# ygahounzo/h-NUMO

Measured on AMD Instinct MI355X. Metric: DG element-updates/sec (all layers, per RK stage), higher is better.
Workload: dtype f64; 1 GPU; dg25L3: double-gyre-3 25x25 elements per GPU, N=4, 3 layers, N_btp=20, kstages=5; elements=625, elements_per_gpu=625, nlayers=3, nop=4, parallelism=single, summation=reference

## Files before the change

### h-numo_amd/csrc/engine.hip

```cpp
#include <hip/hip_runtime.h>
#include <hip/hip_ext.h>

#include <rccl/rccl.h>

#include <algorithm>
#include <cmath>
#include <condition_variable>
#include <cstdio>
#include <cstring>
#include <mutex>
#include <string>
#include <thread>
#include <type_traits>
#include <vector>

#include "../../include/hnumo_engine.h"
#include "engine_internal.h"
#include "setup_plan.h"
#include "sample_plan.h"
#include "float_plan.h"
#include "kernels_bcl.hip"
#include "kernels_btp.hip"
#include "kernels_lapq.hip"
#include "kernels_diag.hip"
// ... 46 lines not shown
  DevMesh m{};
  hnumo_params p{};
  int nelem, npoin, npq, nface, ngl, nq, L, P, Q, K;
  size_t FQ, FN;
  std::vector<void *> allocs;
  double *basis, *qstat, *nstat, *fstat, *fnstat, *alpha, *tau_wind;
  int *iconn;
  std::vector<double> ssprk_a, ssprk_beta;
  double *q, *qb, *qp, *q2, *qp2, *qbp, *qf, *qf2, *qfa, *dpp2;
  double *qbuf[4], *gtrace[2];
  double *qcoef, *ncoef, *fcoef, *fncoef, *dpp_graduv, *dpprime_visc, *gdpp_face;
  double *ecoef, *efcoef;
  double *qstatE, *nstatE, *efstat;
  std::vector<int> fslotA;
  double *qacc, *facc, *nacc, *gfacc, *tau_wind_ave;
  double *slmf, *slmf_face, *dpp, *fmass, *fcons, *momL, *lapf, *rhs;
  int *neg_flag, *h_neg;
  hipGraph_t graph = nullptr;
  hipGraphExec_t graph_exec = nullptr;
  bool resident = false, uploaded = false, alloc_failed = false;
  hipEvent_t ev0 = nullptr, ev1 = nullptr;
  hipEvent_t evk0 = nullptr, evk1 = nullptr;
  bool capturing = false, kernel_events = false, no_graph = false;
  int graph_env = -1;
  int summation = HNUMO_SUM_REFERENCE;
  unsigned long long *stage_prof = nullptr;
  int stage_dbg = 0;
  int stage_nb = 0;
  bool bcl_big = false;
  bool acc_zero = false;
  bool persistent_ok[2] = {false, false};
  bool regacc[2] = {false, false};
  TraceGranule *gtr[2] = {nullptr, nullptr};
  unsigned long long *epoch = nullptr;
  unsigned *sub_done = nullptr;
  unsigned *sub_arrive = nullptr;
  unsigned *steps_done = nullptr, *h_steps = nullptr;
  int occ_blocks[2] = {0, 0}, occ_ncu = 0, probe_ok[2] = {-1, -1};
  int persist_pad = 0;
  int persist_guard = 3;
  int persist_aborts = 0;
  bool persist_suspended = false;
  int persist_wait = 0, persist_backoff = 1, persist_reprobes = 0, persist_recovered = 0;
  unsigned long long *dbg_abort_epoch = nullptr;
  StageArgs *d_stages[2] = {nullptr, nullptr};
  bool face_halo = false;
  int NS = 0;
  using FNbr = SetupPlan::FNbr;
  std::vector<FNbr> fnb;
  int *d_sface = nullptr;
  double *bx_sbuf = nullptr, *bx_rbuf = nullptr;
  size_t bx_per_max = 0;
  int *d_elB = nullptr, *d_elI = nullptr;
  int nB = 0, nI = 0;
  double *cdef = nullptr;
  bool emu_frozen = false;
  int xseq = 0;
  struct Frozen {
    const void *key;
    size_t n;
    double *buf;
  };
  std::vector<Frozen> frozen;
  hipStream_t stream2 = nullptr;
  hipEvent_t ev_fork = nullptr, ev_join = nullptr, ev_I = nullptr, ev_B[2] = {nullptr, nullptr};
  hipEvent_t ev_Is = nullptr, ev_Bs[2] = {nullptr, nullptr};
  hipEvent_t ev_tsent = nullptr, ev_bpacked = nullptr, ev_bdone = nullptr;
  bool lapq_on = false;
  double *dpq = nullptr;
// ... 110 lines not shown
      if (e->summation == HNUMO_SUM_REFERENCE && (e->stage_nb == 4 || e->stage_nb == 5)) {
        if (e->stage_nb == 5)
          launch_nb<5>(n, st, stop, a);
        else
          launch_nb<4>(n, st, stop, a);
        return;
      }
    }
    if (e->summation == HNUMO_SUM_REFERENCE)
      hipLaunchKernelGGL((btp_stage_kernel<NGL, NQ, false>), dim3(n), dim3(StageCfg<NGL, NQ, false>::BS), 0, st, a);
    else
      hipLaunchKernelGGL((btp_stage_kernel<NGL, NQ, true>), dim3(n), dim3(StageCfg<NGL, NQ, true>::BS), 0, st, a);
    if (stop) (void)hipEventRecord(stop, st);
  }
  template <int NB>
  static void launch_nb(int n, hipStream_t st, hipEvent_t stop, const StageArgs &a) {
    if (a.accumulate == 2)
      launch_nb_acc<NB, 1>(n, st, stop, a);
    else if (a.accumulate == 1)
      launch_nb_acc<NB, 2>(n, st, stop, a);
    else
      launch_nb_acc<NB, 0>(n, st, stop, a);
  }
  template <int NB, int ACCF>
  static void launch_nb_acc(int n, hipStream_t st, hipEvent_t stop, const StageArgs &a) {
    using K = StageCfg<NGL, NQ, false, NB>;
    if (stop)
      hipExtLaunchKernelGGL((btp_stage_kernel<NGL, NQ, false, NB, ACCF>), dim3(n), dim3(K::BS), 0, st, nullptr, stop, 0,
                            a);
    else
      hipLaunchKernelGGL((btp_stage_kernel<NGL, NQ, false, NB, ACCF>), dim3(n), dim3(K::BS), 0, st, a);
  }
  static void subcycle(hnumo_engine *e, const StageArgs *stages, int ns) {
    launch_sub(e, e->summation, SubArgs{stages, ns, e->epoch, e->sub_done, e->sub_arrive, e->neg_flag, e->dbg_abort_epoch,
                                        e->d_eperm});
  }
  static void launch_sub(hnumo_engine *e, int sum, const SubArgs &sa) {
    if (sum == HNUMO_SUM_REFERENCE)
      hipLaunchKernelGGL((btp_subcycle_kernel<NGL, NQ, false>), dim3(e->nelem_owned),
                         dim3(StageCfg<NGL, NQ, false>::BS), e->persist_pad, e->stream, sa);
    else
      hipLaunchKernelGGL((btp_subcycle_kernel<NGL, NQ, true>), dim3(e->nelem_owned), dim3(StageCfg<NGL, NQ, true>::BS),
                         e->persist_pad, e->stream, sa);
  }
  static void occupancy(hnumo_engine *e, int ncu) {
    int nb0 = 0, nb1 = 0;
    (void)hipOccupancyMaxActiveBlocksPerMultiprocessor(&nb0, btp_subcycle_kernel<NGL, NQ, false>,
                                                       StageCfg<NGL, NQ, false>::BS, e->persist_pad);
    (void)hipOccupancyMaxActiveBlocksPerMultiprocessor(&nb1, btp_subcycle_kernel<NGL, NQ, true>,
                                                       StageCfg<NGL, NQ, true>::BS, e->persist_pad);
    (void)hipGetLastError();
    e->occ_blocks[0] = nb0;
    e->occ_blocks[1] = nb1;
    e->occ_ncu = ncu;
    const bool est = e->persist_guard & 1;
    const bool persist_slots_ok = (long)e->nelem * 32 * NGL <= (1L << 18);
    e->persistent_ok[0] = persist_slots_ok && (!est || (long)nb0 * ncu >= e->nelem_owned);
    e->persistent_ok[1] = persist_slots_ok && (!est || (long)nb1 * ncu >= e->nelem_owned);
    e->regacc[0] = StageCfg<NGL, NQ, false>::REGACC;
    e->regacc[1] = StageCfg<NGL, NQ, true>::REGACC;
  }
  static void probe(hnumo_engine *e, int sum) {
    launch_sub(e, sum, SubArgs{e->d_stages[0], 0, e->epoch, e->sub_done, e->sub_arrive, e->neg_flag, nullptr, e->d_eperm});
  }
  static void grad_trace(hnumo_engine *e, const double *qb, double *gt, int e0, int n) {
    if (n > 0) {
      hipLaunchKernelGGL((grad_trace_kernel<NGL, NQ>), dim3(n), dim3(64), 0, e->stream, e->m, qb, gt, e0);
      kmark(e, "grad_trace");
    }
  }
  static void extract(hnumo_engine *e, const double *qp, double *qf, int only_dp) {
    size_t n = (size_t)e->nface * NGL;
    hipLaunchKernelGGL((extract_face_kernel<NGL>), dim3((n + 255) / 256), dim3(256), 0, e->stream, e->m, qp, qf,
                       only_dp);
    kmark(e, "extract_face");
    face_exchange_qf(e, qf, only_dp ? 1 : 3);
  }
  static void bcl_coeffs(hnumo_engine *e, double *qp, double *qf, const double *qp_avg = nullptr,
                         const double *qf_avg = nullptr, double *qf_out = nullptr) {
    const bool fz = fused_extract(e);
    hipLaunchKernelGGL((bcl_coeffs_elem_kernel<NGL, NQ>), dim3(e->nelem), dim3(Blk<NGL, NQ>::BSW), 0, e->stream, e->m, qp,
                       qp_avg, e->qcoef, e->ncoef, e->dpp_graduv, e->dpprime_visc, e->ecoef, fz ? qf : nullptr,
                       qf_avg, qf_out, e->fcoef, e->fncoef, e->gdpp_face, e->efcoef);
    kmark(e, "bcl_coeffs_elem");
    if (!fz)
      hipLaunchKernelGGL((bcl_coeffs_face_kernel<NGL, NQ>), dim3(e->nface), dim3(64), 0, e->stream, e->m, qf, qf_avg,
                         e->dpp_graduv, e->dpprime_visc, e->fcoef, e->fncoef, e->gdpp_face, e->efcoef);
    if (!fz) kmark(e, "bcl_coeffs_face");
    if (e->face_halo) {
      face_exchange_gdpp(e);
      if (e->NS)
        hipLaunchKernelGGL((bcl_coeffs_proc_kernel<NGL, NQ>), dim3((e->NS * NGL + 63) / 64), dim3(64), 0, e->stream, e->m,
                         e->gdpp_face, e->d_sface, e->NS, e->fncoef, e->efcoef);
    }
    if (e->lapq_on)
      hipLaunchKernelGGL((lapq_dpp_kernel<NGL, NQ>), dim3(std::min<size_t>(((size_t)e->L * e->npq + 255) / 256, 4096)),
// ... 706 lines not shown
      nb.sbuf = dalloc<double>(eng, nb.nsend * per_max);
      nb.rbuf = dalloc<double>(eng, nb.nrecv * per_max);
      if (eng->alloc_failed) return fail(eng, HNUMO_ERR_DEVICE, "hipMalloc failed (halo buffers)");
      eng->nbh.push_back(nb);
    }
    return init_rccl(eng, halo);
  }
  return 0;
}

static void fill_devmesh(hnumo_engine *eng, const SetupPlan &pl) {
  DevMesh &m = eng->m;
  const hnumo_params &par = eng->p;
  const SetupPlan::ConnOff &o = pl.off;
  m.nelem = eng->nelem; m.npoin = eng->npoin; m.npoin_q = eng->npq; m.nface = eng->nface; m.ngl = eng->ngl;
  m.nq = eng->nq; m.L = eng->L;
  m.efaces = eng->iconn + o.efaces; m.eside = eng->iconn + o.eside; m.ebc = eng->iconn + o.ebc; m.efmap = eng->iconn + o.efmap;
  m.enbr_node = eng->iconn + o.enbr_node; m.enbr_e = eng->iconn + o.enbr_e; m.enbr_lf = eng->iconn + o.enbr_lf;
  m.fnodeL = eng->iconn + o.fnodeL; m.fnodeR = eng->iconn + o.fnodeR; m.fel = eng->iconn + o.fel; m.fer = eng->iconn + o.fer;
  m.fslotL = eng->iconn + o.fslotL; m.fslotR = eng->iconn + o.fslotR; m.fslotA = eng->iconn + o.fslotA;
  m.erec = eng->iconn + o.erec;
  m.qstatE = eng->qstatE; m.nstatE = eng->nstatE; m.efstat = eng->efstat;
  m.basis = eng->basis; m.basis_pd = eng->basis + pl.nb0; m.qstat = eng->qstat; m.nstat = eng->nstat; m.fstat = eng->fstat; m.fnstat = eng->fnstat;
  m.alpha = eng->alpha;
  m.gravity = par.gravity; m.cd = par.cd_mlswe; m.visc = par.visc_mlswe; m.dt = par.dt; m.dt_btp = par.dt_btp;
  m.botfr = par.botfr;
  m.ad = par.ad_mlswe; m.max_shear_dz = par.max_shear_dz; m.shear_corr = par.shear_corrector;
  m.runflag = eng->neg_flag;
  m.steps_done = eng->steps_done;
}

static int setup_persistent(hnumo_engine *eng, const SetupPlan &pl, const Knobs &k, int ncu) {
  const int E = eng->nelem, ngl = eng->ngl;
  eng->epoch = dalloc<unsigned long long>(eng, 1);
  eng->qsv = dalloc<double>(eng, (size_t)E * 8 * ngl * ngl);
  eng->sub_done = dalloc<unsigned>(eng, 1);
  eng->sub_arrive = dalloc<unsigned>(eng, 1);
  eng->dbg_abort_epoch = dalloc<unsigned long long>(eng, 1);
  if (eng->dbg_abort_epoch) HIPCHK(hipMemset(eng->dbg_abort_epoch, 0xff, sizeof(unsigned long long)));
  for (int b = 0; b < 2; b++) eng->gtr[b] = dalloc<TraceGranule>(eng, (size_t)E * 32 * ngl);
  if (k.persist_on) DISPATCH(eng, occupancy(eng, ncu));
  if (k.place) {
    const auto ebc = pl.conn.begin() + pl.off.ebc;
    HIPCHK(dupload(eng, placement_perm(std::vector<int>(ebc, ebc + 4 * E), E, ncu), eng->d_eperm));
    if (k.glue_perm) eng->m.eperm = eng->d_eperm;
  }
  const double *qps[2] = {eng->qp, eng->qp2};
  for (int v = 0; v < 2; v++) {
    std::vector<StageArgs> st;
    (void)stage_table(eng, qps[v], st);
    st.front().qb_in = eng->qb;
    st.front().self_trace = 1;
    st.back().qb_out = v == 0 ? eng->qbp : eng->qb;
    HIPCHK(dupload(eng, st, eng->d_stages[v]));
    if (eng->alloc_failed) return fail(eng, HNUMO_ERR_DEVICE, "hipMalloc failed (stage tables)");
  }
  if (k.persist_on) {
    for (int sm = 0; sm < 2 && (eng->persist_guard & 2); sm++) {
      if (!eng->persistent_ok[sm] || eng->comm_mode != 0 || eng->nranks != 1) continue;
      HIPCHK(hipMemsetAsync(eng->neg_flag, 0, sizeof(int), eng->stream));
      DISPATCH(eng, probe(eng, sm));
      HIPCHK(hipMemcpyAsync(eng->h_neg, eng->neg_flag, sizeof(int), hipMemcpyDeviceToHost, eng->stream));
      HIPCHK(hipStreamSynchronize(eng->stream));
      HIPCHK(hipGetLastError());
      eng->probe_ok[sm] = (*eng->h_neg & RUN_ABORT) ? 0 : 1;
      if (!eng->probe_ok[sm]) eng->persistent_ok[sm] = false;
      HIPCHK(hipMemsetAsync(eng->neg_flag, 0, sizeof(int), eng->stream));
    }
  }
  return 0;
// ... 288 lines not shown
    default: break;
  }
  (void)hipGetLastError();
  const int32_t v[8] = {use_persistent(eng) ? 1 : 0, eng->occ_blocks[0], eng->occ_blocks[1], eng->occ_ncu,
                        eng->probe_ok[0], eng->probe_ok[1], eng->persist_aborts, lds};
  std::memcpy(out, v, sizeof(v));
  return 0;
}

int hnumo_persistent_stats(hnumo_engine *eng, int32_t *out4) {
  if (!eng || !out4) return HNUMO_ERR_INVALID;
  const int32_t v[4] = {eng->persist_aborts, eng->persist_reprobes, eng->persist_recovered,
                        eng->persist_suspended ? eng->persist_wait : -1};
  std::memcpy(out4, v, sizeof(v));
  return 0;
}

int hnumo_debug_frozen_halo(hnumo_engine *eng, int on) {
  if (!eng) return HNUMO_ERR_INVALID;
  if (!eng->face_halo || eng->nranks != 1) {
    eng->err = "the frozen halo is for self-neighbour engines (one-rank processor-face halo) only";
    return HNUMO_ERR_INVALID;
  }
  eng->emu_frozen = on != 0;
  return HNUMO_OK;
}

int hnumo_debug_force_abort(hnumo_engine *eng, int k) {
  if (!eng || k < 0) return HNUMO_ERR_INVALID;
  if (!eng->dbg_abort_epoch) return fail(eng, HNUMO_ERR_INVALID, "engine has no persistent sub-cycle");
  HIPCHK(hipSetDevice(eng->device));
  HIPCHK(hipStreamSynchronize(eng->stream));
  unsigned long long ep = 0;
  HIPCHK(hipMemcpy(&ep, eng->epoch, sizeof(ep), hipMemcpyDeviceToHost));
  ep += (unsigned long long)k;
  HIPCHK(hipMemcpy(eng->dbg_abort_epoch, &ep, sizeof(ep), hipMemcpyHostToDevice));
  return 0;
}

#if HNUMO_BCL_PROF
int hnumo_bcl_prof(unsigned long long *dst, int n) {
  const size_t bytes = std::min<size_t>((size_t)n, 4 * 8192 * 8) * sizeof(unsigned long long);
  return hipMemcpyFromSymbol(dst, HIP_SYMBOL(g_bcl_prof), bytes, 0, hipMemcpyDeviceToHost) == hipSuccess ? 0 : -1;
}
#endif

int hnumo_sync(hnumo_engine *eng, double *q_df, double *qb_df, double *qprime_df) {
  if (!eng) return HNUMO_ERR_INVALID;
  HIPCHK(hipSetDevice(eng->device));
  return download_state(eng, q_df, qb_df, qprime_df);
}

static DiagArgs diag_args(const hnumo_engine *eng) {
  DiagArgs a{};
  a.q = eng->q;
  a.qb = eng->qb;
  a.zbot = eng->nstat + (size_t)NS_ZB * eng->npoin;
  a.alpha = eng->alpha;
  a.cdx = eng->diag_cdx;
  a.cdy = eng->diag_cdy;
  a.gravity = eng->p.gravity;
  a.dt = eng->p.dt;
  a.dt_btp = eng->p.dt_btp;
  a.npoin = eng->npoin;
  a.ne = eng->diag_ne;
  a.ngl = eng->ngl;
  return a;
// ... 651 lines not shown
```

### h-numo_amd/csrc/kernels_btp.hip

```cpp
#include "engine_internal.h"

constexpr int OTF_MIN_NGL = 8;
#define OTF_UNROLL 3
constexpr int PRIO_B = 1, PRIO_S = 2, PRIO_E = 3;
#define DBG(bit) (HNUMO_DIAG && (a.dbg & (bit)))
#define PROF (HNUMO_DIAG && a.prof)
#define SETPRIO_IF(cond, hi, lo)        \
  do {                                  \
    if (cond)                           \
      __builtin_amdgcn_s_setprio(hi);   \
    else                                \
      __builtin_amdgcn_s_setprio(lo);   \
  } while (0)
namespace hnumo {

struct alignas(16) TraceGranule {
  double v;
  unsigned long long tag;
};
__device__ __forceinline__ void st_granule(TraceGranule *p, double v, unsigned long long tag) {
  typedef unsigned u4 __attribute__((ext_vector_type(4)));
  u4 x;
  const unsigned long long vb = __builtin_bit_cast(unsigned long long, v);
  x[0] = (unsigned)vb;
  x[1] = (unsigned)(vb >> 32);
  x[2] = (unsigned)tag;
  x[3] = (unsigned)(tag >> 32);
  asm volatile("global_store_dwordx4 %0, %1, off sc1" ::"v"(p), "v"(x) : "memory");
}
typedef unsigned granule_u4 __attribute__((ext_vector_type(4)));
__device__ __forceinline__ void ld_granule(const TraceGranule *p, double &v, unsigned long long &tag) {
  typedef unsigned u4 __attribute__((ext_vector_type(4)));
  u4 x;
// ... 5 lines not shown
  if (first)
    *p = 0.0 + x;
  else
    atomicAdd(p, x);
}
struct StageArgs {
  DevMesh m;
  const double *qb_in, *qb0, *qb2, *qprime;
  const double *ecoef;
  const double *efcoef;
  const double *trace_in;
  double *trace_out;
  double *qacc, *facc, *nacc, *gfacc;
  double *qb_out;
  double *rhs_out;
  double a1, a2, a3, dtt;
  int rhs_only, write_trace, accumulate;
  unsigned long long *prof;
  int dbg;
  TraceGranule *gtr_in, *gtr_out;
  unsigned long long tag_in, tag_out;
  int first_of_step, save_q2;
  int *err;
  const double *lapq;
  const int *elist;
  int tcontig;
  double *qpq;
  int qpq_mode;
  double *qsv;
  double n_inv;
  int self_trace;
};

typedef __attribute__((address_space(3))) void lds_void_t;
typedef __attribute__((address_space(1))) void glb_void_t;

__device__ __forceinline__ int4 slot_ids4(const int *p) {
  typedef unsigned u4v __attribute__((ext_vector_type(4)));
  u4v t;
  asm volatile("s_load_dwordx4 %0, %1, 0x0\n\ts_waitcnt lgkmcnt(0)" : "=s"(t) : "s"(p));
  return make_int4((int)t.x, (int)t.y, (int)t.z, (int)t.w);
}

template <int BS, bool G16 = false>
__device__ __forceinline__ void glds_copy(const void *g, void *l, int ndw, int tid, int &rot) {
  constexpr int NW = BS / 64;
  const int wave = tid >> 6, lane = tid & 63;
  int d0 = 0;
  if (G16 && (((uintptr_t)g | (uintptr_t)l) & 15) == 0) {
    const int n4 = ndw >> 2;
    const int nch = (n4 + 63) >> 6;
    int c = (wave - rot) % NW;
    if (c < 0) c += NW;
    for (; c < nch; c += NW) {
      const int i = (c << 6) + lane;
      if (i < n4)
        __builtin_amdgcn_global_load_lds((glb_void_t *)((const uint4 *)g + i), (lds_void_t *)((uint4 *)l + (c << 6)),
                                         16, 0, 0);
    }
    rot = (rot + nch) % NW;
    d0 = n4 << 2;
  }
  const int nch = (ndw - d0 + 63) >> 6;
  int c = (wave - rot) % NW;
  if (c < 0) c += NW;
  for (; c < nch; c += NW) {
// ... 128 lines not shown
  }
}

template <int BS, class F>
__device__ __forceinline__ void for_tasks(int tid, int o, int n, F &&f) {
  static_assert((BS & (BS - 1)) == 0, "BS must be a power of two");
  for (int t = (tid - o) & (BS - 1); t < n; t += BS) {
    asm volatile("" ::: "memory");
    f(t, o + t < BS);
  }
}

template <int NGL>
__device__ __forceinline__ void wall_ghost(int er, const double *efn, int n, double &u, double &v) {
  if (er == -4) {
    const double nxn = efn[EFN_NX * NGL + n], nyn = efn[EFN_NY * NGL + n];
    const double un = nxn * u + nyn * v;
    u = u - 2.0 * un * nxn;
    v = v - 2.0 * un * nyn;
  } else if (er == -2) {
    u = -u;
    v = -v;
  }
}

#define STAGE_MARK(k) \
  if (PROF && tid == 0) s_prof[k] = clock64();

#define LDS_BARRIER() asm volatile("s_waitcnt lgkmcnt(0)\n\ts_barrier" ::: "memory")

template <int NGL, int NQ, bool SF, bool PERSIST, class ARGS, int NB = 0, int ACCF = 0, int FST = 0>
__device__ __forceinline__ void stage_body(const ARGS &a, double *s_arena, unsigned long long *s_prof,
                                           const int e, const int tid, unsigned long long ep = 0,
                                           double *pacc = nullptr, int *gdesc = nullptr) {
  static_assert(PERSIST ? (FST == 1 || FST == 2) : FST == 0, "FST is the persistent stage position");
  const int accm = ACCF == 1 ? 2 : (ACCF == 2 ? 1 : a.accumulate);
  constexpr bool first = FST != 2;
  using C = StageCfg<NGL, NQ, SF, NB>;
  constexpr bool REGACC = PERSIST && C::REGACC;
  constexpr int P = C::P, Q = C::Q, BS = C::BS, NCH = C::NCH, QC = C::QC, QCP = C::QCP;
  const auto &m = a.m;
  const int npoin = m.npoin;
  double *const S = s_arena;
  const double *s_psiq = S + C::O_BASIS, *s_dpsiq = s_psiq + NGL * NQ, *s_dpsi = s_dpsiq + NGL * NQ;
  auto PSQ = [&](int x) -> double { return s_psiq[2 * x]; };
  auto DPSQ = [&](int x) -> double { return s_psiq[2 * x + 1]; };
  auto PDQ = [&](int x, double &pv, double &dv) {
    const double2 w = reinterpret_cast<const double2 *>(s_psiq)[x];
    pv = w.x;
    dv = w.y;
  };
  const int *s_er = reinterpret_cast<const int *>(S + C::O_EREC);
  const int *s_side = s_er + EREC_SIDE, *s_bc = s_er + EREC_BC;
  const int *s_nbe = s_er + EREC_NBE, *s_nblf = s_er + EREC_NBLF, *s_map = s_er + EREC_MAP, *s_pf = s_er + EREC_PF(NGL);
  const int *s_acc = s_er + EREC_ACC;
  double *s_qb = S + C::O_QB, *s_q0 = S + C::O_Q0, *s_q2 = S + C::O_Q2;
  double *s_qk = S + C::O_QK;
  double *s_ns = S + C::O_NS;
  double *s_nc = S + C::O_NC;
  double *s_u = S + C::O_UV, *s_v = s_u + P;
  double *s_wn = S + C::O_WN;
  double *s_qv = S + C::O_QV;
  double *s_pq = s_qv + 4 * Q;
  auto QSL = [&](int sl, int q) -> double & { return s_qv[((sl >> 1) * Q + q) * 2 + (sl & 1)]; };
  auto QI = [&](int c, int q) -> double & { return C::SLIM ? QSL(c, q) : s_qv[c * Q + q]; };
  auto QP = [&](int c, int q) -> double & { return C::SLIM ? QSL(4 + c, q) : s_pq[c * Q + q]; };
  auto QO = [&](int k, int q) -> double & { return C::SLIM ? QSL(1 + k, q) : s_qv[k * Q + q]; };
// ... 53 lines not shown
    }
    if (!PERSIST || first) {
      if (m.botfr && qpm != 2)
        glds_copy<BS, C::G16>(a.qprime + (size_t)(m.L - 1) * 3 * npoin + (size_t)e * 3 * P, s_qp, 6 * P, tid, rot);
      glds_copy<BS, C::G16>(m.efstat + (size_t)e * 4 * C::FBLK, s_ef, 2 * 4 * C::FBLK, tid, rot);
      glds_copy<BS, C::G16>(a.efcoef + (size_t)e * 4 * C::EFC, s_ec, 2 * 4 * C::EFC, tid, rot);
    }
  }
  if constexpr (PERSIST) {
    if (first)
      for (int t = tid; t < 4 * P; t += BS) s_qb[t] = a.qb_in[(size_t)e * 4 * P + t];
  }
  constexpr int NST = QE_N - QE_KEEP, NPRE = NST + 7;
  double pre[NPRE];
  double r_wq = 0.0;
  auto load_pre = [&]() {
    if (tid < Q) {
      const double *qse = m.qstatE + (size_t)e * qe_stride(Q) + tid;
      if (C::SLIM) r_wq = qse[0];
#pragma unroll
      for (int k = 0; k < NST; k++) pre[k] = qse[(QE_KEEP + k) * Q];
      const double *eco = a.ecoef + (size_t)e * C::ECO + tid;
#pragma unroll
      for (int k = 0; k < 4; k++) pre[NST + k] = eco[k * Q];
      if (qpm == 2) {
        const double *qq = a.qpq + (size_t)e * 3 * Q + tid;
#pragma unroll
        for (int k = 0; k < 3; k++) pre[NST + 4 + k] = qq[k * Q];
      }
    }
  };
  if (!PERSIST || first) {
    load_pre();
    __syncthreads();
  } else {
    if constexpr (C::SLIM) {
      asm volatile("s_waitcnt vmcnt(0)" ::: "memory");
      LDS_BARRIER();
    }
    load_pre();
  }
  STAGE_MARK(21);
  if constexpr (C::SLIM && PERSIST) {
    if ((a.first_of_step || a.save_q2) && tid >= C::EW * 64 && tid - C::EW * 64 < P) {
      const int p = tid - C::EW * 64;
      double *d = a.qsv + (size_t)e * 8 * P + p * 4;
#pragma unroll
      for (int v = 1; v < 4; v++) {
        const double x = s_qb[p * 4 + v];
        if (a.first_of_step) d[v] = x;
        if (a.save_q2) d[4 * P + v] = x;
      }
    }
  }

  if (tid == 0) S[C::O_BASIS + C::NB] = 0.0;

  static_assert(32 * NGL <= BS, "at most one granule per thread (issue_granule, poll_traces)");
  granule_u4 gx = {0u, 0u, 0u, 0u};
  bool gwant = false;
  constexpr bool GDESC = PERSIST && !C::SLIM && NGL <= 6;
  constexpr int GD_SRC = 13, GD_SLOT = 18;
  int gd = -1;
  if constexpr (GDESC) {
    static_assert(INPL, "the trace source of the new state is s_qb");
    static_assert(C::ARENA <= (1 << GD_SRC), "arena word index in GD_SRC bits");
    static_assert(GD_SRC + GD_SLOT == 31, "the sign bit marks a face without neighbour");
// ... 1148 lines not shown
      if (PERSIST) {
        if (first) s_prof[24] = s_prof[25] = s_prof[26] = s_prof[27] = s_prof[8] = s_prof[9] = s_prof[10] = s_prof[11] = s_prof[29] = 0;
        if (!C::SLIM) s_prof[23] = first ? s_prof[28] : s_prof[23] + s_prof[28];
        s_prof[8] += s_prof[1] - s_prof[21];
        s_prof[9] += s_prof[2] - s_prof[1];
        s_prof[10] += s_prof[3] - s_prof[2];
        s_prof[11] += s_prof[5] - s_prof[3];
        if (C::SLIM)
          s_prof[29] += s_prof[28] - s_prof[2];
        else
          s_prof[29] += s_prof[5] - s_prof[4];
        s_prof[27] += s_prof[22];
        s_prof[24] += s_prof[21] - s_prof[0];
        s_prof[25] += s_prof[5] - s_prof[21];
        s_prof[26] += 1;
      }
      s_prof[31] = wall_clock64();
      for (int k = 0; k < 32; k++) a.prof[(size_t)e * 32 + k] = s_prof[k];
      if (PERSIST) s_prof[22] = 0;
      if (PERSIST && !C::SLIM) s_prof[28] = 0;
    }
  }
}

template <int NGL, int NQ, bool SF, int NB = 0, int ACCF = 0>
__global__ void __launch_bounds__((StageCfg<NGL, NQ, SF, NB>::BS), (StageCfg<NGL, NQ, SF, NB>::MINW))
    btp_stage_kernel(StageArgs a) {
  __shared__ __attribute__((aligned(16))) double s_arena[StageCfg<NGL, NQ, SF, NB>::ARENA];
  __shared__ unsigned long long s_prof[HNUMO_DIAG ? 32 : 1];
  stage_body<NGL, NQ, SF, false, StageArgs, NB, ACCF>(a, s_arena, s_prof,
                                                      a.elist ? a.elist[blockIdx.x] : (int)blockIdx.x, threadIdx.x);
}

struct SubArgs {
  const StageArgs *stages;
  int NS;
  unsigned long long *epoch;
  unsigned *done;
  unsigned *arrive;
  int *err;
  const unsigned long long *abort_epoch;
  const int *eperm;
};

constexpr unsigned RDV_ABORT = 0x80000000u;
constexpr unsigned long long RDV_TICKS = 2000000ull;
__device__ __forceinline__ bool residency_rendezvous(unsigned *arrive, int *err, unsigned grid) {
  if (__hip_atomic_load(err, __ATOMIC_RELAXED, __HIP_MEMORY_SCOPE_AGENT) & RUN_ABORT) return false;
  const unsigned old = __hip_atomic_fetch_add(arrive, 1u, __ATOMIC_RELAXED, __HIP_MEMORY_SCOPE_AGENT);
  if (old & RDV_ABORT) return false;
  if (old + 1 == grid) return true;
  const unsigned long long t0 = wall_clock64();
  for (;;) {
    unsigned w = __hip_atomic_load(arrive, __ATOMIC_RELAXED, __HIP_MEMORY_SCOPE_AGENT);
    if (w & RDV_ABORT) return false;
    if (w == grid) return true;
    if (wall_clock64() - t0 > RDV_TICKS &&
        __hip_atomic_compare_exchange_strong(arrive, &w, w | RDV_ABORT, __ATOMIC_RELAXED, __ATOMIC_RELAXED,
                                             __HIP_MEMORY_SCOPE_AGENT)) {
      __hip_atomic_fetch_or(err, RUN_ABORT, __ATOMIC_RELAXED, __HIP_MEMORY_SCOPE_AGENT);
      return false;
    }
    __builtin_amdgcn_s_sleep(8);
  }
}

template <int NGL, int NQ, bool SF>
__global__ void __launch_bounds__((StageCfg<NGL, NQ, SF>::BS), (StageCfg<NGL, NQ, SF>::MINW))
    btp_subcycle_kernel(SubArgs sa) {
  using C = StageCfg<NGL, NQ, SF>;
  __shared__ __attribute__((aligned(16))) double s_arena[C::ARENA];
  __shared__ unsigned long long s_prof[HNUMO_DIAG ? 32 : 1];
  const int e = sa.eperm ? __builtin_amdgcn_readfirstlane(sa.eperm[blockIdx.x]) : (int)blockIdx.x, tid = threadIdx.x;
  const unsigned long long ep = *sa.epoch;
  typedef const __attribute__((address_space(4))) StageArgs CStageArgs;
  CStageArgs *tab = (CStageArgs *)sa.stages;
  __shared__ int s_go;
  if (tid == 0) {
    if (sa.abort_epoch && *sa.abort_epoch == ep) {
      __hip_atomic_fetch_or(sa.arrive, RDV_ABORT, __ATOMIC_RELAXED, __HIP_MEMORY_SCOPE_AGENT);
      __hip_atomic_fetch_or(sa.err, RUN_ABORT, __ATOMIC_RELAXED, __HIP_MEMORY_SCOPE_AGENT);
      s_go = 0;
    } else {
      s_go = residency_rendezvous(sa.arrive, sa.err, gridDim.x);
    }
  }
  __syncthreads();
  const int NS = s_go ? sa.NS : 0;
  double pacc[16];
#pragma unroll
  for (int k = 0; k < 16; k++) pacc[k] = 0.0;
  int gdesc = -1;
  if (NS > 0) {
    int tid_s = tid, e_s = e;
    asm volatile("" : "+v"(tid_s), "+s"(e_s));
    tid_s &= C::BS - 1;
    stage_body<NGL, NQ, SF, true, CStageArgs, 0, 0, 1>(tab[0], s_arena, s_prof, e_s, tid_s, ep, pacc, &gdesc);
  }
#pragma unroll 1
  for (int stage = 1; stage < NS; stage++) {
    if constexpr (C::SLIM)
      __syncthreads();
    else
      LDS_BARRIER();
    int tid_s = tid, e_s = e;
    asm volatile("" : "+v"(tid_s), "+s"(e_s));
    tid_s &= C::BS - 1;
    stage_body<NGL, NQ, SF, true, CStageArgs, 0, 0, 2>(tab[stage], s_arena, s_prof, e_s, tid_s, ep, pacc, &gdesc);
  }
  if (tid == 0) {
    const unsigned prev = __hip_atomic_fetch_add(sa.done, 1u, __ATOMIC_RELAXED, __HIP_MEMORY_SCOPE_AGENT);
    if (prev == gridDim.x - 1) {
      __hip_atomic_store(sa.epoch, ep + 1, __ATOMIC_RELAXED, __HIP_MEMORY_SCOPE_AGENT);
      __hip_atomic_store(sa.arrive, 0u, __ATOMIC_RELAXED, __HIP_MEMORY_SCOPE_AGENT);
      __hip_atomic_store(sa.done, 0u, __ATOMIC_RELAXED, __HIP_MEMORY_SCOPE_AGENT);
    }
  }
}

template <int NGL, int NQ>
__global__ void __launch_bounds__(64) grad_trace_kernel(DevMesh m, const double *qb, double *trace, int e0) {
  constexpr int P = NGL * NGL, ERS = EREC_SIZE(NGL);
  const int e = e0 + blockIdx.x, tid = threadIdx.x;
  __shared__ double s_dpsi[NGL * NGL + 1], s_qb[P * 4], s_nm[4 * P], s_u[P], s_v[P];
  __shared__ int s_er[ERS];
  for (int t = tid; t < NGL * NGL; t += 64) s_dpsi[t] = m.basis[2 * NGL * NQ + t];
  if (tid == 0) s_dpsi[NGL * NGL] = 0.0;
  for (int t = tid; t < ERS; t += 64) s_er[t] = m.erec[(size_t)e * ERS + t];
  for (int t = tid; t < 4 * P; t += 64) s_qb[t] = qb[(size_t)e * 4 * P + t];
  for (int t = tid; t < 4 * P; t += 64) s_nm[t] = m.nstatE[(size_t)e * NE_N * P + t];
  __syncthreads();
  for (int p = tid; p < P; p += 64) {
    s_u[p] = s_qb[p * 4 + 2] / s_qb[p * 4];
    s_v[p] = s_qb[p * 4 + 3] / s_qb[p * 4];
  }
  __syncthreads();
  for (int t = tid; t < 4 * 8 * NGL; t += 64) {
    const int lf = t / (8 * NGL), c = (t / NGL) % 8, n = t % NGL;
    if (s_er[EREC_BC + lf] < 0) continue;
    const int p = s_er[EREC_MAP + lf * NGL + n];
    double val;
    if (c < 4) {
      val = s_qb[p * 4 + c];
    } else {
      const int cg = c - 4, i = p % NGL, j = p / NGL;
      const double ex = s_nm[((cg & 1) ? NE_EY : NE_EX) * P + p], nx = s_nm[((cg & 1) ? NE_NY : NE_NX) * P + p];
      val = nodal_grad<NGL>(s_dpsi, i, j, ex, nx, (cg >> 1) ? s_v : s_u);
    }
    const size_t slot = (((size_t)s_er[EREC_NBE + lf] * 4 + s_er[EREC_NBLF + lf]) * 8 + c) * NGL + n;
    trace[slot] = val;
// ... 32 lines not shown
```

Measured before the change: 58.87 million element-updates/s.

## Shard residency rendezvous counters and overlap arrival with first-stage prefetch

```diff
diff --git a/h-numo_amd/csrc/engine.hip b/h-numo_amd/csrc/engine.hip
--- a/h-numo_amd/csrc/engine.hip
+++ b/h-numo_amd/csrc/engine.hip
@@ -102,9 +102,7 @@
   bool persistent_ok[2] = {false, false};
   bool regacc[2] = {false, false};
   TraceGranule *gtr[2] = {nullptr, nullptr};
-  unsigned long long *epoch = nullptr;
-  unsigned *sub_done = nullptr;
-  unsigned *sub_arrive = nullptr;
+  ResidencyBlock *res = nullptr;
   unsigned *steps_done = nullptr, *h_steps = nullptr;
   int occ_blocks[2] = {0, 0}, occ_ncu = 0, probe_ok[2] = {-1, -1};
   int persist_pad = 0;
@@ -281,8 +279,7 @@
       hipLaunchKernelGGL((btp_stage_kernel<NGL, NQ, false, NB, ACCF>), dim3(n), dim3(K::BS), 0, st, a);
   }
   static void subcycle(hnumo_engine *e, const StageArgs *stages, int ns) {
-    launch_sub(e, e->summation, SubArgs{stages, ns, e->epoch, e->sub_done, e->sub_arrive, e->neg_flag, e->dbg_abort_epoch,
-                                        e->d_eperm});
+    launch_sub(e, e->summation, SubArgs{stages, ns, e->res, e->neg_flag, e->dbg_abort_epoch, e->d_eperm, 0});
   }
   static void launch_sub(hnumo_engine *e, int sum, const SubArgs &sa) {
     if (sum == HNUMO_SUM_REFERENCE)
@@ -310,7 +307,9 @@
     e->regacc[1] = StageCfg<NGL, NQ, true>::REGACC;
   }
   static void probe(hnumo_engine *e, int sum) {
-    launch_sub(e, sum, SubArgs{e->d_stages[0], 0, e->epoch, e->sub_done, e->sub_arrive, e->neg_flag, nullptr, e->d_eperm});
+    const int dbg = HNUMO_DIAG ? e->stage_dbg & (8192 | 16384) : 0;
+    launch_sub(e, sum, SubArgs{e->d_stages[0], 0, e->res, e->neg_flag, nullptr, e->d_eperm, dbg});
+    if (dbg & 16384) (void)hipMemsetAsync(e->res, 0, offsetof(ResidencyBlock, epoch), e->stream);
   }
   static void grad_trace(hnumo_engine *e, const double *qb, double *gt, int e0, int n) {
     if (n > 0) {
@@ -1083,10 +1082,8 @@
 
 static int setup_persistent(hnumo_engine *eng, const SetupPlan &pl, const Knobs &k, int ncu) {
   const int E = eng->nelem, ngl = eng->ngl;
-  eng->epoch = dalloc<unsigned long long>(eng, 1);
+  eng->res = dalloc<ResidencyBlock>(eng, 1);
   eng->qsv = dalloc<double>(eng, (size_t)E * 8 * ngl * ngl);
-  eng->sub_done = dalloc<unsigned>(eng, 1);
-  eng->sub_arrive = dalloc<unsigned>(eng, 1);
   eng->dbg_abort_epoch = dalloc<unsigned long long>(eng, 1);
   if (eng->dbg_abort_epoch) HIPCHK(hipMemset(eng->dbg_abort_epoch, 0xff, sizeof(unsigned long long)));
   for (int b = 0; b < 2; b++) eng->gtr[b] = dalloc<TraceGranule>(eng, (size_t)E * 32 * ngl);
@@ -1441,7 +1438,7 @@
   HIPCHK(hipSetDevice(eng->device));
   HIPCHK(hipStreamSynchronize(eng->stream));
   unsigned long long ep = 0;
-  HIPCHK(hipMemcpy(&ep, eng->epoch, sizeof(ep), hipMemcpyDeviceToHost));
+  HIPCHK(hipMemcpy(&ep, &eng->res->epoch.v, sizeof(ep), hipMemcpyDeviceToHost));
   ep += (unsigned long long)k;
   HIPCHK(hipMemcpy(eng->dbg_abort_epoch, &ep, sizeof(ep), hipMemcpyHostToDevice));
   return 0;
diff --git a/h-numo_amd/csrc/kernels_btp.hip b/h-numo_amd/csrc/kernels_btp.hip
--- a/h-numo_amd/csrc/kernels_btp.hip
+++ b/h-numo_amd/csrc/kernels_btp.hip
@@ -1,4 +1,5 @@
 #include "engine_internal.h"
+#include "residency.h"
 
 constexpr int OTF_MIN_NGL = 8;
 #define OTF_UNROLL 3
@@ -70,6 +71,27 @@
   int self_trace;
 };
 
+struct SubArgs {
+  const StageArgs *stages;
+  int NS;
+  ResidencyBlock *res;
+  int *err;
+  const unsigned long long *abort_epoch;
+  const int *eperm;
+  int dbg;
+};
+
+__device__ __forceinline__ bool subcycle_arrive(const SubArgs &sa, unsigned long long ep) {
+  if (HNUMO_DIAG && (sa.dbg & 8192)) return true;
+  if (sa.abort_epoch && *sa.abort_epoch == ep) {
+    res_force_abort(sa.res, sa.err, RUN_ABORT);
+    return false;
+  }
+  return res_arrive(
+      sa.res, sa.err, RUN_ABORT, gridDim.x, blockIdx.x, [] { return (unsigned long long)wall_clock64(); },
+      [] { __builtin_amdgcn_s_sleep(8); });
+}
+
 typedef __attribute__((address_space(3))) void lds_void_t;
 typedef __attribute__((address_space(1))) void glb_void_t;
 
@@ -264,7 +286,8 @@
 template <int NGL, int NQ, bool SF, bool PERSIST, class ARGS, int NB = 0, int ACCF = 0, int FST = 0>
 __device__ __forceinline__ void stage_body(const ARGS &a, double *s_arena, unsigned long long *s_prof,
                                            const int e, const int tid, unsigned long long ep = 0,
-                                           double *pacc = nullptr, int *gdesc = nullptr) {
+                                           double *pacc = nullptr, int *gdesc = nullptr,
+                                           const SubArgs *gate = nullptr, int *s_go = nullptr) {
   static_assert(PERSIST ? (FST == 1 || FST == 2) : FST == 0, "FST is the persistent stage position");
   const int accm = ACCF == 1 ? 2 : (ACCF == 2 ? 1 : a.accumulate);
   constexpr bool first = FST != 2;
@@ -384,7 +407,15 @@
   };
   if (!PERSIST || first) {
     load_pre();
+    if constexpr (FST == 1)
+      if (gate && tid == 0) *s_go = subcycle_arrive(*gate, ep);
     __syncthreads();
+    if constexpr (FST == 1) {
+      if (gate && !*s_go) {
+        asm volatile("s_waitcnt vmcnt(0)" ::: "memory");
+        return;
+      }
+    }
   } else {
     if constexpr (C::SLIM) {
       asm volatile("s_waitcnt vmcnt(0)" ::: "memory");
@@ -1599,39 +1630,6 @@
                                                       a.elist ? a.elist[blockIdx.x] : (int)blockIdx.x, threadIdx.x);
 }
 
-struct SubArgs {
-  const StageArgs *stages;
-  int NS;
-  unsigned long long *epoch;
-  unsigned *done;
-  unsigned *arrive;
-  int *err;
-  const unsigned long long *abort_epoch;
-  const int *eperm;
-};
-
-constexpr unsigned RDV_ABORT = 0x80000000u;
-constexpr unsigned long long RDV_TICKS = 2000000ull;
-__device__ __forceinline__ bool residency_rendezvous(unsigned *arrive, int *err, unsigned grid) {
-  if (__hip_atomic_load(err, __ATOMIC_RELAXED, __HIP_MEMORY_SCOPE_AGENT) & RUN_ABORT) return false;
-  const unsigned old = __hip_atomic_fetch_add(arrive, 1u, __ATOMIC_RELAXED, __HIP_MEMORY_SCOPE_AGENT);
-  if (old & RDV_ABORT) return false;
-  if (old + 1 == grid) return true;
-  const unsigned long long t0 = wall_clock64();
-  for (;;) {
-    unsigned w = __hip_atomic_load(arrive, __ATOMIC_RELAXED, __HIP_MEMORY_SCOPE_AGENT);
-    if (w & RDV_ABORT) return false;
-    if (w == grid) return true;
-    if (wall_clock64() - t0 > RDV_TICKS &&
-        __hip_atomic_compare_exchange_strong(arrive, &w, w | RDV_ABORT, __ATOMIC_RELAXED, __ATOMIC_RELAXED,
-                                             __HIP_MEMORY_SCOPE_AGENT)) {
-      __hip_atomic_fetch_or(err, RUN_ABORT, __ATOMIC_RELAXED, __HIP_MEMORY_SCOPE_AGENT);
-      return false;
-    }
-    __builtin_amdgcn_s_sleep(8);
-  }
-}
-
 template <int NGL, int NQ, bool SF>
 __global__ void __launch_bounds__((StageCfg<NGL, NQ, SF>::BS), (StageCfg<NGL, NQ, SF>::MINW))
     btp_subcycle_kernel(SubArgs sa) {
@@ -1639,31 +1637,27 @@
   __shared__ __attribute__((aligned(16))) double s_arena[C::ARENA];
   __shared__ unsigned long long s_prof[HNUMO_DIAG ? 32 : 1];
   const int e = sa.eperm ? __builtin_amdgcn_readfirstlane(sa.eperm[blockIdx.x]) : (int)blockIdx.x, tid = threadIdx.x;
-  const unsigned long long ep = *sa.epoch;
+  const unsigned long long ep = sa.res->epoch.v;
   typedef const __attribute__((address_space(4))) StageArgs CStageArgs;
   CStageArgs *tab = (CStageArgs *)sa.stages;
   __shared__ int s_go;
-  if (tid == 0) {
-    if (sa.abort_epoch && *sa.abort_epoch == ep) {
-      __hip_atomic_fetch_or(sa.arrive, RDV_ABORT, __ATOMIC_RELAXED, __HIP_MEMORY_SCOPE_AGENT);
-      __hip_atomic_fetch_or(sa.err, RUN_ABORT, __ATOMIC_RELAXED, __HIP_MEMORY_SCOPE_AGENT);
-      s_go = 0;
-    } else {
-      s_go = residency_rendezvous(sa.arrive, sa.err, gridDim.x);
-    }
-  }
-  __syncthreads();
-  const int NS = s_go ? sa.NS : 0;
   double pacc[16];
 #pragma unroll
   for (int k = 0; k < 16; k++) pacc[k] = 0.0;
   int gdesc = -1;
-  if (NS > 0) {
+  constexpr bool HOIST = NGL < 8;
+  if (!HOIST || sa.NS == 0) {
+    if (tid == 0) s_go = subcycle_arrive(sa, ep);
+    __syncthreads();
+  }
+  if (sa.NS > 0 && (HOIST || s_go)) {
     int tid_s = tid, e_s = e;
     asm volatile("" : "+v"(tid_s), "+s"(e_s));
     tid_s &= C::BS - 1;
-    stage_body<NGL, NQ, SF, true, CStageArgs, 0, 0, 1>(tab[0], s_arena, s_prof, e_s, tid_s, ep, pacc, &gdesc);
-  }
+    stage_body<NGL, NQ, SF, true, CStageArgs, 0, 0, 1>(tab[0], s_arena, s_prof, e_s, tid_s, ep, pacc, &gdesc,
+                                                       HOIST ? &sa : nullptr, &s_go);
+  }
+  const int NS = s_go ? sa.NS : 0;
 #pragma unroll 1
   for (int stage = 1; stage < NS; stage++) {
     if constexpr (C::SLIM)
@@ -1675,14 +1669,7 @@
     tid_s &= C::BS - 1;
     stage_body<NGL, NQ, SF, true, CStageArgs, 0, 0, 2>(tab[stage], s_arena, s_prof, e_s, tid_s, ep, pacc, &gdesc);
   }
-  if (tid == 0) {
-    const unsigned prev = __hip_atomic_fetch_add(sa.done, 1u, __ATOMIC_RELAXED, __HIP_MEMORY_SCOPE_AGENT);
-    if (prev == gridDim.x - 1) {
-      __hip_atomic_store(sa.epoch, ep + 1, __ATOMIC_RELAXED, __HIP_MEMORY_SCOPE_AGENT);
-      __hip_atomic_store(sa.arrive, 0u, __ATOMIC_RELAXED, __HIP_MEMORY_SCOPE_AGENT);
-      __hip_atomic_store(sa.done, 0u, __ATOMIC_RELAXED, __HIP_MEMORY_SCOPE_AGENT);
-    }
-  }
+  if (tid == 0 && !(HNUMO_DIAG && (sa.dbg & 16384))) (void)res_leave(sa.res, gridDim.x, blockIdx.x, ep);
 }
 
 template <int NGL, int NQ>
diff --git a/h-numo_amd/csrc/residency.h b/h-numo_amd/csrc/residency.h
--- /dev/null
+++ b/h-numo_amd/csrc/residency.h
@@ -0,0 +1,105 @@
+#pragma once
+#include <stdint.h>
+
+#if defined(__HIPCC__)
+#define HNUMO_RES_HD __host__ __device__
+#else
+#define HNUMO_RES_HD
+#endif
+
+namespace hnumo {
+
+constexpr unsigned RES_SHARDS = 8;
+constexpr unsigned RES_ABORT = 0x80000000u;
+constexpr unsigned long long RES_TICKS = 2000000ull;
+
+struct alignas(128) ResidencyWord {
+  unsigned v;
+  unsigned pad[31];
+};
+struct alignas(128) ResidencyEpoch {
+  unsigned long long v;
+  unsigned long long pad[15];
+};
+struct ResidencyBlock {
+  ResidencyWord arrive[RES_SHARDS], top, leave[RES_SHARDS], out;
+  ResidencyEpoch epoch;
+};
+static_assert(sizeof(ResidencyWord) == 128 && sizeof(ResidencyEpoch) == 128, "a line per word");
+static_assert(sizeof(ResidencyBlock) == 128 * (2 * RES_SHARDS + 3), "no padding but the words' own");
+
+#if defined(__HIP_DEVICE_COMPILE__)
+#define HNUMO_RES_AT(op, ...) __hip_atomic_##op(__VA_ARGS__, __ATOMIC_RELAXED, __HIP_MEMORY_SCOPE_AGENT)
+HNUMO_RES_HD inline unsigned res_load(const unsigned *p) { return HNUMO_RES_AT(load, p); }
+HNUMO_RES_HD inline int res_load(const int *p) { return HNUMO_RES_AT(load, p); }
+HNUMO_RES_HD inline void res_store(unsigned *p, unsigned v) { HNUMO_RES_AT(store, p, v); }
+HNUMO_RES_HD inline void res_store(unsigned long long *p, unsigned long long v) { HNUMO_RES_AT(store, p, v); }
+HNUMO_RES_HD inline unsigned res_add(unsigned *p, unsigned v) { return HNUMO_RES_AT(fetch_add, p, v); }
+HNUMO_RES_HD inline void res_or(unsigned *p, unsigned v) { (void)HNUMO_RES_AT(fetch_or, p, v); }
+HNUMO_RES_HD inline void res_or(int *p, int v) { (void)HNUMO_RES_AT(fetch_or, p, v); }
+HNUMO_RES_HD inline bool res_cas(unsigned *p, unsigned &expect, unsigned v) {
+  return __hip_atomic_compare_exchange_strong(p, &expect, v, __ATOMIC_RELAXED, __ATOMIC_RELAXED,
+                                              __HIP_MEMORY_SCOPE_AGENT);
+}
+#undef HNUMO_RES_AT
+#else
+HNUMO_RES_HD inline unsigned res_load(const unsigned *p) { return __atomic_load_n(p, __ATOMIC_RELAXED); }
+HNUMO_RES_HD inline int res_load(const int *p) { return __atomic_load_n(p, __ATOMIC_RELAXED); }
+HNUMO_RES_HD inline void res_store(unsigned *p, unsigned v) { __atomic_store_n(p, v, __ATOMIC_RELAXED); }
+HNUMO_RES_HD inline void res_store(unsigned long long *p, unsigned long long v) { __atomic_store_n(p, v, __ATOMIC_RELAXED); }
+HNUMO_RES_HD inline unsigned res_add(unsigned *p, unsigned v) { return __atomic_fetch_add(p, v, __ATOMIC_RELAXED); }
+HNUMO_RES_HD inline void res_or(unsigned *p, unsigned v) { (void)__atomic_fetch_or(p, v, __ATOMIC_RELAXED); }
+HNUMO_RES_HD inline void res_or(int *p, int v) { (void)__atomic_fetch_or(p, v, __ATOMIC_RELAXED); }
+HNUMO_RES_HD inline bool res_cas(unsigned *p, unsigned &expect, unsigned v) {
+  return __atomic_compare_exchange_n(p, &expect, v, false, __ATOMIC_RELAXED, __ATOMIC_RELAXED);
+}
+#endif
+
+HNUMO_RES_HD inline unsigned res_expect(unsigned grid, unsigned s) {
+  return grid / RES_SHARDS + (s < grid % RES_SHARDS ? 1u : 0u);
+}
+HNUMO_RES_HD inline unsigned res_shards(unsigned grid) { return grid < RES_SHARDS ? grid : RES_SHARDS; }
+
+template <class CLOCK, class PAUSE>
+HNUMO_RES_HD inline bool res_arrive(ResidencyBlock *b, int *err, int run_abort, unsigned grid, unsigned wg, CLOCK clock,
+                                    PAUSE pause) {
+  if (res_load(err) & run_abort) return false;
+  const unsigned s = wg % RES_SHARDS, full = res_shards(grid);
+  if (res_add(&b->arrive[s].v, 1u) + 1 == res_expect(grid, s)) {
+    const unsigned old = res_add(&b->top.v, 1u);
+    if (old & RES_ABORT) return false;
+    if (old + 1 == full) return true;
+  }
+  const unsigned long long t0 = clock();
+  for (;;) {
+    unsigned w = res_load(&b->top.v);
+    if (w & RES_ABORT) return false;
+    if (w == full) return true;
+    if (clock() - t0 > RES_TICKS && res_cas(&b->top.v, w, w | RES_ABORT)) {
+      res_or(err, run_abort);
+      return false;
+    }
+    pause();
+  }
+}
+
+HNUMO_RES_HD inline void res_force_abort(ResidencyBlock *b, int *err, int run_abort) {
+  res_or(&b->top.v, RES_ABORT);
+  res_or(err, run_abort);
+}
+
+HNUMO_RES_HD inline bool res_leave(ResidencyBlock *b, unsigned grid, unsigned wg, unsigned long long ep) {
+  const unsigned s = wg % RES_SHARDS;
+  if (res_add(&b->leave[s].v, 1u) + 1 != res_expect(grid, s)) return false;
+  if (res_add(&b->out.v, 1u) + 1 != res_shards(grid)) return false;
+  res_store(&b->epoch.v, ep + 1);
+  for (unsigned k = 0; k < RES_SHARDS; k++) {
+    res_store(&b->arrive[k].v, 0u);
+    res_store(&b->leave[k].v, 0u);
+  }
+  res_store(&b->top.v, 0u);
+  res_store(&b->out.v, 0u);
+  return true;
+}
+
+}
```

Measured after the change: 59.30 million element-updates/s (median of 6 runs). No clear change (+0.7%).
